# DLR-AMR/t8gpu

Hardware: AMD Instinct MI355X
Metric: M cell-updates/sec (flux+RK3 step) on Kelvin-Helmholtz AMR (higher is better)
Workload: dtype f64

## Files before the change

### include/t8gpu_hip.h

```cpp
#ifndef T8GPU_HIP_H
#define T8GPU_HIP_H

#include <stddef.h>
#include <stdint.h>

#ifdef __cplusplus
extern "C" {
#endif

#define T8GPU_FLUX_KEPES 0
#define T8GPU_FLUX_HLL 1
#define T8GPU_FLUX_HLLC 2

typedef struct T8gpuVars_f32 { float* p[5]; } T8gpuVars_f32;
typedef struct T8gpuVars_f64 { double* p[5]; } T8gpuVars_f64;

int         t8gpu_hip_abi_version(void);
int         t8gpu_hip_device_count(int* count);
int         t8gpu_hip_set_device(int device);
const char* t8gpu_hip_error_string(int code);
int         t8gpu_hip_range_push(const char* name);
int         t8gpu_hip_range_pop(void);
const char* t8gpu_hip_last_stage_kernel(void);

// ... 48 lines not shown
                                   void* stream);
int t8gpu_hip_subgrid_boundary_f64(int flux_kind, int rank, int num_faces, int num_boundary_faces,
                                   const int32_t* face_neighbors, const double* face_normals,
                                   const double* face_surfaces, T8gpuVars_f64 state, T8gpuVars_f64 fluxes,
                                   void* stream);
int t8gpu_hip_subgrid_boundary_bc_f32(int flux_kind, int rank, int num_faces, int num_boundary_faces,
                                      const int32_t* face_neighbors, const uint8_t* boundary_kinds, const float* inflow_table,
                                      const float* face_normals, const float* face_surfaces, T8gpuVars_f32 state,
                                      T8gpuVars_f32 fluxes, void* stream);
int t8gpu_hip_subgrid_boundary_bc_f64(int flux_kind, int rank, int num_faces, int num_boundary_faces,
                                      const int32_t* face_neighbors, const uint8_t* boundary_kinds, const double* inflow_table,
                                      const double* face_normals, const double* face_surfaces, T8gpuVars_f64 state,
                                      T8gpuVars_f64 fluxes, void* stream);
int t8gpu_hip_subgrid_boundary_far_f32(int flux_kind, int rank, int num_faces, int num_boundary_faces,
                                       const int32_t* face_neighbors, const uint8_t* boundary_kinds, const float* inflow_table,
                                       const float* face_normals, const float* face_surfaces, T8gpuVars_f32 state,
                                       T8gpuVars_f32 fluxes, void* stream);
int t8gpu_hip_subgrid_boundary_far_f64(int flux_kind, int rank, int num_faces, int num_boundary_faces,
                                       const int32_t* face_neighbors, const uint8_t* boundary_kinds, const double* inflow_table,
                                       const double* face_normals, const double* face_surfaces, T8gpuVars_f64 state,
                                       T8gpuVars_f64 fluxes, void* stream);

int t8gpu_hip_subgrid_rk3_stage_f32(int stage, int rank, int num_elements, T8gpuVars_f32 prev, T8gpuVars_f32 mid,
                                    T8gpuVars_f32 out, T8gpuVars_f32 fluxes, const float* volumes, float delta_t,
                                    void* stream);
int t8gpu_hip_subgrid_rk3_stage_f64(int stage, int rank, int num_elements, T8gpuVars_f64 prev, T8gpuVars_f64 mid,
                                    T8gpuVars_f64 out, T8gpuVars_f64 fluxes, const double* volumes, double delta_t,
                                    void* stream);

typedef struct T8gpuPlainPlan {
  const int32_t*  elem_off;
  const int32_t*  halo_off;
  const int32_t*  face_off;
  const int32_t*  halo_ids;
  const uint32_t* face_lr;
  const void*     face_geo;
  const int32_t*  face_orig;
  const int32_t*  csr_off;
  const uint16_t* csr_ent;
  const int32_t*  tile_order;
  int32_t ntiles, n_interior_tiles, max_elems, max_halo, max_faces, ell_width;
  const uint16_t* ell;
  const uint16_t* geo_idx;
  const void*     geo_table;
  int32_t n_geo;
  int32_t max_slots;
  int32_t n_deep_tiles;
  int32_t n_slots_addressed;
  const int32_t* tile_desc;
  int32_t n_patch_tiles[3];
  int32_t patch_dim;
  int32_t n_irregular_tiles[3];
  const void*    ghost_buf;
  const int32_t* send_map;
  const int32_t* send_list;
  void*          send_buf;
  int32_t        n_owned;
  int32_t        reserved7;
  const void*    inflow;
  int32_t        has_open_faces;
  int32_t        has_farfield_faces;
} T8gpuPlainPlan;

#define T8GPU_INFLOW_WORDS 16
int t8gpu_hip_plain_inflow_table_f32(const float* states, int num_states, float* table, void* stream);
int t8gpu_hip_plain_inflow_table_f64(const double* states, int num_states, double* table, void* stream);

int t8gpu_hip_plain_fused_stage_f32(int flux_kind, int stage, const T8gpuPlainPlan* plan, int tile_begin,
                                    int tile_count, T8gpuVars_f32 prev, T8gpuVars_f32 mid, T8gpuVars_f32 out,
                                    const float* volume, float delta_t, float* speed_estimates, void* stream);
int t8gpu_hip_plain_fused_stage_f64(int flux_kind, int stage, const T8gpuPlainPlan* plan, int tile_begin,
                                    int tile_count, T8gpuVars_f64 prev, T8gpuVars_f64 mid, T8gpuVars_f64 out,
                                    const double* volume, double delta_t, double* speed_estimates, void* stream);

int t8gpu_hip_plain_fused_stage_planar_f32(int flux_kind, int stage, const T8gpuPlainPlan* plan, int tile_begin,
                                           int tile_count, T8gpuVars_f32 prev, T8gpuVars_f32 mid, T8gpuVars_f32 out,
                                           const float* volume, float delta_t, float* speed_estimates, void* stream, int planar);
int t8gpu_hip_plain_fused_stage_planar_f64(int flux_kind, int stage, const T8gpuPlainPlan* plan, int tile_begin,
                                           int tile_count, T8gpuVars_f64 prev, T8gpuVars_f64 mid, T8gpuVars_f64 out,
                                           const double* volume, double delta_t, double* speed_estimates, void* stream, int planar);

int t8gpu_hip_plain_persistent_accepts(const T8gpuPlainPlan* plan, int flux_kind, int float_size, int tile_count);
int t8gpu_hip_plain_needs_csr(const T8gpuPlainPlan* plan);
int t8gpu_hip_plain_geo_frames_f32(void* geo_table, int n_geo, void* stream);
int t8gpu_hip_plain_geo_frames_f64(void* geo_table, int n_geo, void* stream);

int t8gpu_hip_halo_pack_f32(int n_send, int cells_per_element, const int32_t* send_idx, T8gpuVars_f32 state,
                            float* sendbuf, void* stream);
int t8gpu_hip_halo_pack_f64(int n_send, int cells_per_element, const int32_t* send_idx, T8gpuVars_f64 state,
                            double* sendbuf, void* stream);
int t8gpu_hip_halo_unpack_f32(int num_ghosts, int first_ghost_slot, int cells_per_element, const float* recvbuf,
                              T8gpuVars_f32 state, void* stream);
int t8gpu_hip_halo_unpack_f64(int num_ghosts, int first_ghost_slot, int cells_per_element, const double* recvbuf,
                              T8gpuVars_f64 state, void* stream);

int t8gpu_hip_comm_unique_id(char* id128);
int t8gpu_hip_comm_create(const char* id128, int rank, int nranks, void** comm);
int t8gpu_hip_comm_destroy(void* comm);
int t8gpu_hip_comm_abort(void* comm);
int t8gpu_hip_stream_wait(void* stream, double timeout_s);
int t8gpu_hip_runtime_versions(int out4[4]);

typedef struct T8gpuHalo {
  int32_t num_elements, num_ghosts, n_peers, n_send;
  int32_t cells_per_element, reserved;
  const int32_t* peers;
  const int32_t* send_off;
  const int32_t* recv_off;
  const int32_t* send_idx;
  void* sendbuf;
  void* recvbuf;
  void* comm;
} T8gpuHalo;

int t8gpu_hip_halo_exchange_f32(const T8gpuHalo* halo, T8gpuVars_f32 state, void* stream);
int t8gpu_hip_halo_exchange_f64(const T8gpuHalo* halo, T8gpuVars_f64 state, void* stream);

int t8gpu_hip_plain_stepper_create(const T8gpuPlainPlan* plan, const T8gpuHalo* halo_or_null, void** stepper);
int t8gpu_hip_plain_stepper_destroy(void* stepper);
int t8gpu_hip_plain_stepper_iterate_f32(void* stepper, int flux_kind, float* planes, size_t stride, int prev, int next,
                                        float delta_t, float* speed_estimates, void* stream);
int t8gpu_hip_plain_stepper_iterate_f64(void* stepper, int flux_kind, double* planes, size_t stride, int prev, int next,
                                        double delta_t, double* speed_estimates, void* stream);
int t8gpu_hip_plain_stepper_iterate_steps_f32(void* stepper, int flux_kind, float* planes, size_t stride, int prev, int next,
                                              float delta_t, float* speed_estimates, int n_steps, void* stream);
int t8gpu_hip_plain_stepper_iterate_steps_f64(void* stepper, int flux_kind, double* planes, size_t stride, int prev, int next,
                                              double delta_t, double* speed_estimates, int n_steps, void* stream);
int t8gpu_hip_plain_stepper_graph(void* stepper, int enable, int* counts);
int t8gpu_hip_plain_stepper_timing(void* stepper, int enable);
int t8gpu_hip_stepper_set_planar(void* stepper, int mode);
int t8gpu_hip_stepper_planar(void* stepper);
int t8gpu_hip_stepper_host_profile(int reset, double* ns4, long long* calls4);
int t8gpu_hip_plain_stepper_elapsed(void* stepper, double* total_ms, int* launches);
int t8gpu_hip_plain_stepper_timed_stages(void* stepper);
int t8gpu_hip_plain_stepper_host_time(void* stepper, int reset, double* total_ms, long long* steps);

typedef struct T8gpuSubgridPlan {
  const int32_t* block_rec;
  const int32_t* bf_rec;
  int32_t num_elements, rank, max_faces_per_block, n_interior_blocks;
  int32_t n_deep_blocks;
  int32_t n_blocks_addressed;
  const int32_t* fam_rec;
  const int32_t* rest_rec;
  int32_t n_families, n_rest;
  const void*    inflow;
  int32_t        has_open_faces;
  int32_t        has_farfield_faces;
} T8gpuSubgridPlan;

int t8gpu_hip_subgrid_fused_stage_f32(int flux_kind, int stage, const T8gpuSubgridPlan* plan, int block_begin,
                                      int block_count, T8gpuVars_f32 prev, T8gpuVars_f32 mid, T8gpuVars_f32 out,
                                      const float* volumes, float delta_t, void* stream);
int t8gpu_hip_subgrid_fused_stage_f64(int flux_kind, int stage, const T8gpuSubgridPlan* plan, int block_begin,
                                      int block_count, T8gpuVars_f64 prev, T8gpuVars_f64 mid, T8gpuVars_f64 out,
                                      const double* volumes, double delta_t, void* stream);

int t8gpu_hip_subgrid_stepper_create(const T8gpuSubgridPlan* plan, const T8gpuHalo* halo_or_null, void** stepper);
int t8gpu_hip_subgrid_stepper_iterate_steps_f32(void* stepper, int flux_kind, float* planes, size_t stride, const float* volumes,
                                                int prev, int next, float delta_t, int n_steps, void* stream);
int t8gpu_hip_subgrid_stepper_iterate_steps_f64(void* stepper, int flux_kind, double* planes, size_t stride, const double* volumes,
                                                int prev, int next, double delta_t, int n_steps, void* stream);

size_t t8gpu_hip_reduce_workspace_bytes(void);
int t8gpu_hip_planes_or_bits_f32(size_t n, const float* const planes[4], uint32_t* out4, void* stream);
int t8gpu_hip_planes_or_bits_f64(size_t n, const double* const planes[4], uint32_t* out4, void* stream);
// ... 81 lines not shown
```

### t8gpu_amd/csrc/hip/fused_common.hpp

```cpp
#ifndef T8GPU_HIP_FUSED_COMMON_HPP
#define T8GPU_HIP_FUSED_COMMON_HPP

#include <hip/hip_runtime.h>

#include <cstdlib>
#include <type_traits>
#include <utility>

#include "flux_math.hpp"
#include "t8gpu_hip.h"

namespace t8gpu_hip {

inline int device_cu_count() {
  static const int n = [] {
    int             dev = 0;
    hipDeviceProp_t prop;
    if (hipGetDevice(&dev) != hipSuccess || hipGetDeviceProperties(&prop, dev) != hipSuccess) return 0;
    return prop.multiProcessorCount > 0 ? prop.multiProcessorCount : 256;
  }();
  return n;
}
inline int env_per_cu(const char* name) {
  const char* env = std::getenv(name);
// ... 203 lines not shown
}
template <class T>
T8_DEV void inflow_prim(const T8gpuPlainPlan& P, int k, Prim<T>& q) {
  const T* w = inflow_entry<T>(P, k) + 5;
  q.rho = w[0]; q.vx = w[1]; q.vy = w[2]; q.vz = w[3]; q.p = w[4]; q.beta = w[5]; q.lrho = w[6]; q.lbeta = w[7]; q.v0 = w[8];
}

template <class T>
struct vec16;
template <>
struct vec16<double> {
  using type = double2;
  static constexpr int lanes = 2;
};
template <>
struct vec16<float> {
  using type = float4;
  static constexpr int lanes = 4;
};

template <class T, int NW>
constexpr int rec_words() {
  return sizeof(T) == 8 ? (NW > 5 ? 10 : 6) : 12;
}

template <class T>
size_t record_lds(int kind, size_t words, size_t records) {
  const size_t rec = kind == 0 ? rec_words<T, kPrimWords>() : rec_words<T, 5>();
  return sizeof(T) * (words + rec * records) + lds_log_table<T>(kind);
}

template <class T, int NW>
T8_DEV void rec_store(T* rec, const T* w) {
  using V         = typename vec16<T>::type;
  constexpr int L = vec16<T>::lanes;
#pragma unroll
  for (int c = 0; c + L <= NW; c += L) {
    V v;
    T* vv = reinterpret_cast<T*>(&v);
#pragma unroll
    for (int j = 0; j < L; j++) vv[j] = w[c + j];
    *reinterpret_cast<V*>(rec + c) = v;
  }
#pragma unroll
  for (int c = NW / L * L; c < NW; c++) rec[c] = w[c];
}

template <class T, int NW>
T8_DEV void rec_load(const T* rec, T* w) {
  using V         = typename vec16<T>::type;
  constexpr int L = vec16<T>::lanes;
#pragma unroll
  for (int c = 0; c + L <= NW; c += L) {
    const V  v  = *reinterpret_cast<const V*>(rec + c);
    const T* vv = reinterpret_cast<const T*>(&v);
#pragma unroll
    for (int j = 0; j < L; j++) w[c + j] = vv[j];
  }
#pragma unroll
  for (int c = NW / L * L; c < NW; c++) w[c] = rec[c];
}

template <class T>
T8_DEV void prim_words(const T s[5], T w[kPrimWords], const double* logtab) {
  const Prim<T> q = prim_from_state<T, sizeof(T) == 8>(s, logtab);
  w[0] = q.rho; w[1] = q.vx; w[2] = q.vy; w[3] = q.vz; w[4] = q.p; w[5] = q.beta; w[6] = q.lrho; w[7] = q.lbeta; w[8] = q.v0;
}
template <class T>
T8_DEV void words_prim(const T w[kPrimWords], Prim<T>& q) {
  q.rho = w[0]; q.vx = w[1]; q.vy = w[2]; q.vz = w[3]; q.p = w[4]; q.beta = w[5]; q.lrho = w[6]; q.lbeta = w[7]; q.v0 = w[8];
}

constexpr int kPrimWordsPlanar = 8;
template <class T>
T8_DEV void prim_words_planar(const T s[4], T w[kPrimWordsPlanar], const double* logtab) {
  const Prim<T> q = prim_from_state_planar<T, sizeof(T) == 8>(s, logtab);
  w[0] = q.rho; w[1] = q.vx; w[2] = q.vy; w[3] = q.p; w[4] = q.beta; w[5] = q.lrho; w[6] = q.lbeta; w[7] = q.v0;
}
template <class T>
T8_DEV void words_prim_planar(const T w[kPrimWordsPlanar], Prim<T>& q) {
  q.rho = w[0]; q.vx = w[1]; q.vy = w[2]; q.p = w[3]; q.beta = w[4]; q.lrho = w[5]; q.lbeta = w[6]; q.v0 = w[7];
}

template <class T>
int plain_persistent_stage(int kind, int stage, const T8gpuPlainPlan* plan, int tile_begin, int tile_count, FVars<T> prev,
                           FVars<T> mid, FVars<T> out, const T* volume, T dt, T* speed, hipStream_t stream);

template <class T>
int plain_patch_stage(int kind, int stage, const T8gpuPlainPlan* plan, int patch_begin, int patch_count, int tile_begin, int tile_count,
                      FVars<T> prev, FVars<T> mid, FVars<T> out, const T* volume, T dt, T* speed, bool persistent, bool planar,
                      hipStream_t stream);

template <class T>
int plain_patch3_stage(int kind, int stage, const T8gpuPlainPlan* plan, int tile_begin, int tile_count, FVars<T> prev, FVars<T> mid,
                       FVars<T> out, const T* volume, T dt, T* speed, bool persistent, bool irregular, hipStream_t stream);

template <class T>
int plain_patch3_both_stage(int kind, int stage, const T8gpuPlainPlan* plan, int reg_begin, int reg_count, int irr_begin, int irr_count,
                            FVars<T> prev, FVars<T> mid, FVars<T> out, const T* volume, T dt, T* speed, hipStream_t stream);

}

#endif
```

### t8gpu_amd/csrc/hip/kernels_compat.hip

```cpp
#include <hip/hip_runtime.h>

#pragma clang fp contract(off)

#include "flux_math.hpp"
#include "fused_common.hpp"
#include "stage_kernel_note.hpp"
#include "t8gpu_hip.h"
#include "t8gpu_host.h"

namespace t8gpu_hip {

template <class T>
struct Vars {
  T* p[5];
};

template <class T>
T8_DEV void load5(const Vars<T>& v, size_t i, T s[5]) {
#pragma unroll
  for (int k = 0; k < 5; k++) s[k] = v.p[k][i];
}

template <class T>
T8_DEV void gadd(T* addr, T v) {
// ... 405 lines not shown
  if (rank == 3) {
    if (kind == 0) T8_INNER(0, 3); else if (kind == 1) T8_INNER(1, 3); else T8_INNER(2, 3);
  } else {
    if (kind == 0) T8_INNER(0, 2); else if (kind == 1) T8_INNER(1, 2); else T8_INNER(2, 2);
  }
#undef T8_INNER
  return launch_status();
}

template <class T, bool WALL, class V>
int subgrid_faces(int kind, int rank, int F, int count, const int32_t* fn, const int32_t* idx, const int32_t* ld,
                  const int32_t* off, const T* normals, const T* areas, V st, V fl, void* stream) {
  if (count <= 0) return 0;
  if ((rank != 2 && rank != 3) || (kind < 0 || kind > 2)) return static_cast<int>(hipErrorInvalidValue);
  hipStream_t s   = static_cast<hipStream_t>(stream);
  const int   fpb = rank == 3 ? 4 : 16;
  const dim3  block(64), grid((count + fpb - 1) / fpb);
#define T8_FACES(K, R)                                                                                              \
  hipLaunchKernelGGL((k_subgrid_faces<T, K, R, WALL>), grid, block, 0, s, F, count, fn, idx, ld, off, normals, areas, \
                     mk<T>(st), mk<T>(fl))
  if (rank == 3) {
    if (kind == 0) T8_FACES(0, 3); else if (kind == 1) T8_FACES(1, 3); else T8_FACES(2, 3);
  } else {
    if (kind == 0) T8_FACES(0, 2); else if (kind == 1) T8_FACES(1, 2); else T8_FACES(2, 2);
  }
#undef T8_FACES
  return launch_status();
}

template <class T, class V>
int subgrid_boundary_bc(int kind, int rank, int F, int B, const int32_t* fn, const uint8_t* kinds, const T* inflow, const T* normals,
                        const T* areas, V st, V fl, void* stream) {
  if (!kinds) return subgrid_faces<T, true, V>(kind, rank, F, B, fn, nullptr, nullptr, nullptr, normals, areas, st, fl, stream);
  if (B <= 0) return 0;
  if ((rank != 2 && rank != 3) || (kind < 0 || kind > 2)) return static_cast<int>(hipErrorInvalidValue);
  hipStream_t s   = static_cast<hipStream_t>(stream);
  const int   fpb = rank == 3 ? 4 : 16;
  const dim3  block(64), grid((B + fpb - 1) / fpb);
#define T8_BC(K, R) \
  hipLaunchKernelGGL((k_subgrid_boundary_bc<T, K, R>), grid, block, 0, s, F, B, fn, kinds, inflow, normals, areas, mk<T>(st), mk<T>(fl))
  if (rank == 3) {
    if (kind == 0) T8_BC(0, 3); else if (kind == 1) T8_BC(1, 3); else T8_BC(2, 3);
  } else {
    if (kind == 0) T8_BC(0, 2); else if (kind == 1) T8_BC(1, 2); else T8_BC(2, 2);
  }
#undef T8_BC
  return launch_status();
}

template <class T, class V>
int subgrid_boundary_far(int kind, int rank, int F, int B, const int32_t* fn, const uint8_t* kinds, const T* inflow, const T* normals,
                         const T* areas, V st, V fl, void* stream) {
  if (!kinds) return subgrid_faces<T, true, V>(kind, rank, F, B, fn, nullptr, nullptr, nullptr, normals, areas, st, fl, stream);
  if (B <= 0) return 0;
  if ((rank != 2 && rank != 3) || (kind < 0 || kind > 2)) return static_cast<int>(hipErrorInvalidValue);
  hipStream_t s   = static_cast<hipStream_t>(stream);
  const int   fpb = rank == 3 ? 4 : 16;
  const dim3  block(64), grid((B + fpb - 1) / fpb);
#define T8_FAR(K, R) \
  hipLaunchKernelGGL((k_subgrid_boundary_far<T, K, R>), grid, block, 0, s, F, B, fn, kinds, inflow, normals, areas, mk<T>(st), mk<T>(fl))
  if (rank == 3) {
    if (kind == 0) T8_FAR(0, 3); else if (kind == 1) T8_FAR(1, 3); else T8_FAR(2, 3);
  } else {
    if (kind == 0) T8_FAR(0, 2); else if (kind == 1) T8_FAR(1, 2); else T8_FAR(2, 2);
  }
#undef T8_FAR
  return launch_status();
}

}

namespace t8gpu_hip {
StageKernelNote& stage_kernel_note() {
  static thread_local StageKernelNote note = {{0}, -1};
  return note;
}
}

using namespace t8gpu_hip;

extern "C" {

const char* t8gpu_hip_last_stage_kernel(void) { return stage_kernel_note().name; }
int t8gpu_hip_abi_version(void) { return 13; }
int t8gpu_hip_device_count(int* count) { return static_cast<int>(hipGetDeviceCount(count)); }
int t8gpu_hip_set_device(int device) { return static_cast<int>(hipSetDevice(device)); }
const char* t8gpu_hip_error_string(int code) {
  if (code >= 10000) return "RCCL error (code - 10000 is the ncclResult_t)";
  return hipGetErrorString(static_cast<hipError_t>(code));
}

#define T8_DEFINE_COMPAT(SUF, T, V)                                                                                  \
  int t8gpu_hip_flux_faces_##SUF(int kind, int F, int ndim, const int32_t* fn, const int32_t* idx, const T* normals, \
                                 const T* areas, V st, V fl, T* speed, void* stream) {                               \
    return flux_faces<T, V>(kind, F, ndim, fn, idx, normals, areas, st, fl, speed, stream);                          \
  }                                                                                                                  \
  int t8gpu_hip_flux_boundary_##SUF(int kind, int F, int B, int ndim, const int32_t* fn, const T* normals,           \
                                    const T* areas, V st, V fl, T* speed, void* stream) {                            \
    return flux_boundary<T, V>(kind, F, B, ndim, fn, normals, areas, st, fl, speed, stream);                         \
  }                                                                                                                  \
  int t8gpu_hip_flux_boundary_bc_##SUF(int kind, int F, int B, int ndim, const int32_t* fn, const uint8_t* kinds,       \
                                       const T* inflow, const T* normals, const T* areas, V st, V fl, T* speed,        \
                                       void* stream) {                                                                 \
    return flux_boundary_bc<T, V>(kind, F, B, ndim, fn, kinds, inflow, normals, areas, st, fl, speed, stream);         \
  }                                                                                                                  \
  int t8gpu_hip_rk3_stage_##SUF(int stage, int N, V prev, V mid, V out, V fl, const T* volume, T dt, void* stream) { \
    return rk_stage<T, 1, V>(stage, N < 0 ? 0 : (size_t)N, prev, mid, out, fl, volume, dt, stream);                  \
  }                                                                                                                  \
  int t8gpu_hip_subgrid_inner_##SUF(int kind, int rank, int N, V st, V fl, const T* volumes, void* stream) {         \
    return subgrid_inner<T, V>(kind, rank, N, st, fl, volumes, stream);                                              \
  }                                                                                                                  \
  int t8gpu_hip_subgrid_outer_##SUF(int kind, int rank, int F, const int32_t* fn, const int32_t* idx,                \
                                    const int32_t* ld, const int32_t* off, const T* normals, const T* areas, V st,   \
                                    V fl, void* stream) {                                                            \
    return subgrid_faces<T, false, V>(kind, rank, F, F, fn, idx, ld, off, normals, areas, st, fl, stream);           \
  }                                                                                                                  \
  int t8gpu_hip_subgrid_boundary_##SUF(int kind, int rank, int F, int B, const int32_t* fn, const T* normals,        \
                                       const T* areas, V st, V fl, void* stream) {                                   \
    return subgrid_faces<T, true, V>(kind, rank, F, B, fn, nullptr, nullptr, nullptr, normals, areas, st, fl,        \
                                     stream);                                                                        \
  }                                                                                                                  \
  int t8gpu_hip_subgrid_boundary_bc_##SUF(int kind, int rank, int F, int B, const int32_t* fn, const uint8_t* kinds,  \
                                          const T* inflow, const T* normals, const T* areas, V st, V fl,             \
                                          void* stream) {                                                            \
    return subgrid_boundary_bc<T, V>(kind, rank, F, B, fn, kinds, inflow, normals, areas, st, fl, stream);           \
  }                                                                                                                  \
  int t8gpu_hip_subgrid_boundary_far_##SUF(int kind, int rank, int F, int B, const int32_t* fn, const uint8_t* kinds, \
                                           const T* inflow, const T* normals, const T* areas, V st, V fl,            \
                                           void* stream) {                                                           \
    return subgrid_boundary_far<T, V>(kind, rank, F, B, fn, kinds, inflow, normals, areas, st, fl, stream);          \
  }                                                                                                                  \
  int t8gpu_hip_subgrid_rk3_stage_##SUF(int stage, int rank, int N, V prev, V mid, V out, V fl, const T* volumes,    \
                                        T dt, void* stream) {                                                        \
    if (rank == 3) return rk_stage<T, 64, V>(stage, (size_t)(N < 0 ? 0 : N) * 64, prev, mid, out, fl, volumes, dt, stream); \
    if (rank == 2) return rk_stage<T, 16, V>(stage, (size_t)(N < 0 ? 0 : N) * 16, prev, mid, out, fl, volumes, dt, stream); \
    return static_cast<int>(hipErrorInvalidValue);                                                                   \
  }

T8_DEFINE_COMPAT(f32, float, T8gpuVars_f32)
T8_DEFINE_COMPAT(f64, double, T8gpuVars_f64)

}
```

### t8gpu_amd/csrc/hip/kernels_fused_patch.hip

```cpp
#include "fused_common.hpp"
#include "fused_tile_body.hpp"
#include "patch_common.hpp"
#include "stage_kernel_note.hpp"

namespace t8gpu_hip {

template <class T, int KIND, int STAGE, bool NT, bool PLANAR = false>
T8_DEV void plain_patch_body(const T8gpuPlainPlan& P, int tile_begin, int tile_count, int wg, int nwg, int chunk, const FVars<T>& prev,
                             const FVars<T>& src, const FVars<T>& out, const T* __restrict__ vol, T dt, T* __restrict__ speed) {
  static_assert(!PLANAR || KIND == 0, "the planar form exists for KEPES");
  constexpr int NV  = PLANAR ? 4 : 5;
  constexpr int NW  = KIND == 0 ? (PLANAR ? kPrimWordsPlanar : kPrimWords) : 5;
  constexpr int REC = rec_words<T, NW>();
  auto pl = [](int c) { return PLANAR && c == 3 ? 4 : c; };
  extern __shared__ __attribute__((aligned(16))) double lds_raw[];
  T* const  ff = reinterpret_cast<T*>(lds_raw);
  T* const  pe = ff + NV * kPatchFF;
  constexpr bool kTab = sizeof(T) == 8 && KIND == 0;
  double* const lt = reinterpret_cast<double*>(pe + REC * 320);
  const int tid = threadIdx.x;

  const int G = nwg, xcd = wg & 7, jw = wg >> 3;
  const int nxcd = G < 8 ? G : 8, nx = (G - xcd + 7) >> 3;
  const int per = tile_count / nxcd, rem = tile_count % nxcd;
  const int x0   = tile_begin + xcd * per + (xcd < rem ? xcd : rem);
  int       tend = x0 + per + (xcd < rem ? 1 : 0);
  int       t    = x0 + (chunk > 0 ? jw * chunk : jw);
  if (chunk > 0 && t + chunk < tend) tend = t + chunk;
  if (xcd >= nxcd || t >= tend) return;
  if (kTab) {
    lt[tid] = kLogTab[tid];
    __syncthreads();
  }

  int ci = 0, cj = 0;
#pragma unroll
  for (int b = 0; b < 4; b++) {
    ci |= ((tid >> (2 * b)) & 1) << b;
    cj |= ((tid >> (2 * b + 1)) & 1) << b;
  }
  const int  rx   = ci < 15 ? patch_morton(ci + 1, cj) : 272 + cj;
  const int  ry   = cj < 15 ? patch_morton(ci, cj + 1) : 304 + ci;
  const int  a_mx = ci > 0 ? patch_morton(ci - 1, cj) : 512 + cj;
  const int  a_my = cj > 0 ? 256 + patch_morton(ci, cj - 1) : 528 + ci;
  const bool yfirst_lane = patch_ctz4(cj) >= patch_ctz4(ci);
  const int  wv = __builtin_amdgcn_readfirstlane(tid >> 6), ln = tid & 63;
  auto role = [&](int it) { return (wv + it) & 3; };
  const int  hl      = ln;
  const bool minus_y = ln >= 16;
  const int  m_l = 256 + (minus_y ? 32 : 0) + (ln & 15);
  const int  m_r = minus_y ? patch_morton(ln & 15, 0) : patch_morton(0, ln & 15);

  typedef int int8v __attribute__((ext_vector_type(8)));
  struct Desc {
    int    e0, h0, fbase, flags;
    double area, vol;
  };
  auto load_desc = [&](int tt) {
    const size_t k = static_cast<size_t>(tt < tend ? tt : tend - 1);
    const int8v  r = *reinterpret_cast<const __attribute__((address_space(4))) int8v*>(
        reinterpret_cast<const __attribute__((address_space(4))) char*>(reinterpret_cast<uintptr_t>(P.tile_desc)) + 32 * k);
    Desc d;
    d.e0 = r[0]; d.h0 = r[2]; d.fbase = r[4]; d.flags = r[5];
    d.area = __hiloint2double(r[7], r[6]);
    d.vol  = __hiloint2double(r[3], r[1]);
    return d;
  };
  struct Pre {
    T s0[NV], sh[NV];
  };
  auto prefetch = [&](const Desc& d, int hslot, bool first, bool halo_wave) {
    Pre p;
#pragma unroll
    for (int k = 0; k < NV; k++) p.s0[k] = at32<T>(src.p[pl(k)], static_cast<unsigned>(d.e0 + tid));
    if (!PLANAR && halo_wave && first && P.ghost_buf) {
#pragma unroll
      for (int k = 0; k < NV; k++) p.sh[k] = ghost_window_load<T>(P, src, hslot, pl(k));
    } else if (halo_wave) {
#pragma unroll
      for (int k = 0; k < NV; k++) p.sh[k] = at32<T>(src.p[pl(k)], static_cast<unsigned>(hslot));
    } else {
#pragma unroll
      for (int k = 0; k < NV; k++) p.sh[k] = T(0);
    }
    return p;
  };

  const int stride = chunk > 0 ? 1 : nx;
  Desc      d0 = load_desc(t), d1 = load_desc(t + stride);
  int       hs_a = role(0) == 3 ? P.halo_ids[d0.h0 + hl] : 0, hs_b = role(1) == 3 ? P.halo_ids[d1.h0 + hl] : 0;
  Pre       cur = prefetch(d0, hs_a, true, role(0) == 3);
  int       it  = 0;
  T         res[NV];
#pragma unroll
  for (int k = 0; k < NV; k++) res[k] = T(0);
  int       res_e  = -1;
  __builtin_amdgcn_s_waitcnt(0);

  for (; t < tend; t += stride, it++) {
    const bool halo_wave = role(it) == 3, minus_lane = role(it) == 0 && ln < 32;
    const Desc d2   = load_desc(t + 2 * stride);
    const int  hs_c = role(it + 2) == 3 ? P.halo_ids[d2.h0 + hl] : 0;
    Pre        nxt;
    if (t + stride < tend) nxt = prefetch(d1, hs_b, false, role(it + 1) == 3);
    const int e = d0.e0 + tid;
    T         pv[NV];
#pragma unroll
    for (int k = 0; k < NV; k++) pv[k] = T(0);
    if (STAGE > 1) {
#pragma unroll
      for (int k = 0; k < NV; k++) pv[k] = stream_load<NT>(&at32<T>(prev.p[pl(k)], static_cast<unsigned>(e)));
    }
    const T volume = (d0.flags & 0x400) ? static_cast<T>(d0.vol) : at32<T>(vol, static_cast<unsigned>(e));
    const T area   = static_cast<T>(d0.area);

    T mine[NW];
    if constexpr (PLANAR) {
      prim_words_planar<T>(cur.s0, mine, lt);
    } else if constexpr (KIND == 0) {
      prim_words<T>(cur.s0, mine, lt);
    } else {
#pragma unroll
      for (int k = 0; k < 5; k++) mine[k] = cur.s0[k];
    }
    rec_store<T, NW>(pe + tid * REC, mine);
    if (halo_wave) {
      T w[NW];
      if constexpr (PLANAR) {
        prim_words_planar<T>(cur.sh, w, lt);
      } else if constexpr (KIND == 0) {
        prim_words<T>(cur.sh, w, lt);
      } else {
#pragma unroll
        for (int k = 0; k < 5; k++) w[k] = cur.sh[k];
      }
      rec_store<T, NW>(pe + (256 + hl) * REC, w);
    }
    if (res_e >= 0) {
#pragma unroll
      for (int k = 0; k < NV; k++) stream_store<NT>(&at32<T>(out.p[pl(k)], static_cast<unsigned>(res_e)), res[k]);
    }
    __syncthreads();

    auto face = [&](bool y, const T* wl, const T* wr, T* g, T& spd) {
      if constexpr (PLANAR)
        patch_face_planar<T>(y, wl, wr, area, g, spd);
      else
        patch_face<T, KIND, NW>(y, wl, wr, area, g, spd);
    };
    T gy[NV];
    {
      T wr[NW], g[NV], sx, sy;
      rec_load<T, NW>(pe + rx * REC, wr);
      face(false, mine, wr, g, sx);
#pragma unroll
      for (int k = 0; k < NV; k++) ff[k * kPatchFF + tid] = g[k];
      rec_load<T, NW>(pe + ry * REC, wr);
      face(true, mine, wr, gy, sy);
#pragma unroll
      for (int k = 0; k < NV; k++) ff[k * kPatchFF + 256 + tid] = gy[k];
      if (speed) {
        T* const sp = speed + d0.fbase + 2 * tid;
        if ((d0.fbase & 1) == 0 || sizeof(T) == 4) {
          using V2 = typename vec2<T>::type;
          V2 v;
          v.x = sx;
          v.y = sy;
          *reinterpret_cast<V2*>(sp) = v;
        } else {
          sp[0] = sx;
          sp[1] = sy;
        }
      }
    }
    if (minus_lane) {
      T wl[NW], wr[NW], g[NV], sm;
      rec_load<T, NW>(pe + m_l * REC, wl);
      rec_load<T, NW>(pe + m_r * REC, wr);
      face(minus_y, wl, wr, g, sm);
#pragma unroll
      for (int k = 0; k < NV; k++) ff[k * kPatchFF + 512 + ln] = g[k];
    }
    __syncthreads();

    const bool yfirst = tid == 0 ? (d0.flags & 1) != 0 : yfirst_lane;
    const int  a1 = yfirst ? a_my : a_mx, a2 = yfirst ? a_mx : a_my;
    T          acc[NV];
#pragma unroll
    for (int k = 0; k < NV; k++) {
      acc[k] = __builtin_fma(T(1), ff[k * kPatchFF + a1], T(0));
      acc[k] = __builtin_fma(T(1), ff[k * kPatchFF + a2], acc[k]);
      acc[k] = __builtin_fma(T(-1), ff[k * kPatchFF + tid], acc[k]);
      acc[k] = __builtin_fma(T(-1), gy[k], acc[k]);
    }
    const T scale = (d0.flags & 0x400) ? rk_scale(dt, static_cast<T>(d0.vol)) : dt / volume;
#pragma unroll
    for (int k = 0; k < NV; k++) res[k] = rk_stage_update<T, STAGE>(pv[k], cur.s0[k], scale, acc[k]);
    res_e = e;

    cur  = nxt;
    d0   = d1;
    d1   = d2;
    hs_b = hs_c;
  }
  if (res_e >= 0) {
#pragma unroll
    for (int k = 0; k < NV; k++) stream_store<NT>(&at32<T>(out.p[pl(k)], static_cast<unsigned>(res_e)), res[k]);
    if constexpr (!PLANAR)
      if (P.send_map) ghost_window_send<T>(P, res_e, res);
  }
}

template <class T, int KIND, int STAGE, bool NT, bool PLANAR = false>
__global__ __launch_bounds__(256, sizeof(T) == 8 ? 3 : 5) void k_plain_patch(T8gpuPlainPlan P, int tile_begin, int tile_count, int chunk, FVars<T> prev,
                                                                                FVars<T> src, FVars<T> out, const T* __restrict__ vol, T dt,
                                                                                T* __restrict__ speed) {
  plain_patch_body<T, KIND, STAGE, NT, PLANAR>(P, tile_begin, tile_count, blockIdx.x, gridDim.x, chunk, prev, src, out, vol, dt, speed);
}

template <class T, int KIND, int STAGE, bool NT, bool OPEN = false, bool PLANAR = false>
__global__ __launch_bounds__(256, sizeof(T) == 8 ? 3 : 5) void k_plain_stage(T8gpuPlainPlan P, int patch_begin, int patch_count, int patch_wgs, int chunk,
                                                                                int tile_begin, int tile_count, FVars<T> prev, FVars<T> src,
                                                                                FVars<T> out, const T* __restrict__ vol, T dt,
                                                                                T* __restrict__ speed) {
  const int b = blockIdx.x;
  if (b < patch_wgs) {
    plain_patch_body<T, KIND, STAGE, NT, PLANAR>(P, patch_begin, patch_count, b, patch_wgs, chunk, prev, src, out, vol, dt, speed);
  } else {
    const int pos = tile_begin + xcd_position(b - patch_wgs, tile_count);
    plain_tile_body<T, KIND, STAGE, true, 2, false, OPEN>(P, pos, prev, src, out, vol, dt, speed);
  }
}

template <class T>
int plain_patch_stage(int kind, int stage, const T8gpuPlainPlan* plan, int patch_begin, int patch_count, int tile_begin, int tile_count,
                      FVars<T> prev, FVars<T> mid, FVars<T> out, const T* volume, T dt, T* speed, bool persistent, bool planar,
                      hipStream_t stream) {
  if (patch_count <= 0) return tile_count > 0 ? -1 : 0;
  const bool shared_gpu = plan->n_interior_tiles < plan->ntiles && patch_count + (tile_count > 0 ? tile_count : 0) < plan->ntiles;
  if (!plan->tile_desc) return static_cast<int>(hipErrorInvalidValue);
  if (!plan_planes_fit_32bit<T>(plan)) return static_cast<int>(hipErrorInvalidValue);
  if (plan->ghost_buf || plan->send_map || !persistent || kind != 0) planar = false;
  size_t lds = record_lds<T>(kind, static_cast<size_t>(planar ? 4 : 5) * kPatchFF, 320);
  if (tile_count > 0 && plan->has_farfield_faces) return -1;
  if (tile_count > 0) {
    if (!plain_tiles_pipelined(plan) || plan->max_faces > 512 || !plan->geo_idx || !plan->geo_table || plan->n_geo <= 0) return -1;
    const int    nw       = kind == 0 ? kPrimWords : 5;
    const size_t tab      = lds_log_table<T>(kind);
    const size_t lds_tile = sizeof(T) * (static_cast<size_t>(nw) * plan_slots(*plan) + static_cast<size_t>(5) * 256) + (tab ? tab + 16 : 0);
    if (lds_tile > lds) lds = lds_tile;
    if (sizeof(T) == 8 && 3 * lds > static_cast<size_t>(156) * 1024) return -1;
  }
  const int cus = device_cu_count();
  if (cus == 0) return static_cast<int>(hipErrorInvalidDevice);
  if (plan->ghost_buf || plan->send_map) persistent = false;
  const int  per_cu    = sizeof(T) == 8 ? 3 : 5;
  const int  resident  = cus * per_cu;
  int chunk = 0;
  if (persistent && shared_gpu && patch_count >= resident) chunk = 3;
  int patch_wgs = (!persistent || patch_count < resident) ? patch_count : resident;
  if (chunk > 0) {
    const int share = (patch_count + 7) / 8;
    patch_wgs       = 8 * ((share + chunk - 1) / chunk);
  }
  const dim3 grid(patch_wgs + (tile_count > 0 ? tile_count : 0)), block(256);
  const bool nt = stream_hint(plan->n_slots_addressed, sizeof(T));
  return dispatch(
      [&](auto K, auto S, auto NT, auto MIXED, auto OPEN, auto PLANAR) {
        constexpr bool PL = PLANAR && K == 0;
        if constexpr (MIXED) {
          note_stage_kernel<T>(patch_count + tile_count, "k_plain_stage", K, S, NT, OPEN, PL);
          return launch(&k_plain_stage<T, K, S, NT, OPEN, PL>, grid, block, lds, stream, *plan, patch_begin, patch_count, patch_wgs, chunk,
                        tile_begin, tile_count, prev, mid, out, volume, dt, speed);
        } else {
          note_stage_kernel<T>(patch_count, "k_plain_patch", K, S, NT, PL);
          return launch(&k_plain_patch<T, K, S, NT, PL>, grid, block, lds, stream, *plan, patch_begin, patch_count, chunk, prev, mid, out, volume,
                        dt, speed);
        }
      },
      kind, stage, nt, tile_count > 0, tile_count > 0 && plan->has_open_faces, planar);
}

template int plain_patch_stage<float>(int, int, const T8gpuPlainPlan*, int, int, int, int, FVars<float>, FVars<float>, FVars<float>,
                                      const float*, float, float*, bool, bool, hipStream_t);
template int plain_patch_stage<double>(int, int, const T8gpuPlainPlan*, int, int, int, int, FVars<double>, FVars<double>, FVars<double>,
                                       const double*, double, double*, bool, bool, hipStream_t);

}
```

### t8gpu_amd/csrc/hip/patch_common.hpp

```cpp
#ifndef T8GPU_HIP_PATCH_COMMON_HPP
#define T8GPU_HIP_PATCH_COMMON_HPP

#include "fused_common.hpp"

namespace t8gpu_hip {

template <class T>
T8_DEV const T& at32(const T* base, unsigned i) {
  return *reinterpret_cast<const T*>(reinterpret_cast<const char*>(base) + i * static_cast<unsigned>(sizeof(T)));
}
template <class T>
T8_DEV T& at32(T* base, unsigned i) {
  return *reinterpret_cast<T*>(reinterpret_cast<char*>(base) + i * static_cast<unsigned>(sizeof(T)));
}

template <class T>
bool plan_planes_fit_32bit(const T8gpuPlainPlan* plan) {
  return plan->n_slots_addressed > 0 && static_cast<unsigned long long>(plan->n_slots_addressed) * sizeof(T) < (1ull << 32);
}

constexpr int kPatchFF = 544;

T8_DEV int patch_morton(int i, int j) {
  int t = 0;
#pragma unroll
  for (int b = 0; b < 4; b++) t |= (((i >> b) & 1) << (2 * b)) | (((j >> b) & 1) << (2 * b + 1));
  return t;
}
T8_DEV int patch_ctz4(int v) { return v == 0 ? 4 : __builtin_ctz(static_cast<unsigned>(v)); }

template <class T>
T8_DEV void frame_in(bool y, T vx, T vy, T vz, T& u, T& v, T& w) {
  u = y ? vy : vx;
  v = y ? vx : -vz;
  w = y ? -vz : vy;
}
template <class T>
T8_DEV void frame_out(bool y, const T f[5], T g[5]) {
  g[0] = f[0];
  g[1] = y ? f[2] : f[1];
  g[2] = y ? f[1] : f[3];
  g[3] = y ? -f[3] : -f[2];
  g[4] = f[4];
}

template <class T, int KIND, int NW>
T8_DEV void patch_face(bool y, const T* wl, const T* wr, T area, T g[5], T& spd) {
  T f[5];
  if (KIND == 0) {
    Prim<T> L, R;
    words_prim<T>(wl, L);
    words_prim<T>(wr, R);
    T uL, vL, wL, uR, vR, wR;
    frame_in<T>(y, L.vx, L.vy, L.vz, uL, vL, wL);
    frame_in<T>(y, R.vx, R.vy, R.vz, uR, vR, wR);
    kepes_core<T>(L, R, uL, vL, wL, uR, vR, wR, area, f, spd);
  } else {
    T a[5], b[5];
    a[0] = wl[0]; a[4] = wl[4];
    b[0] = wr[0]; b[4] = wr[4];
    frame_in<T>(y, wl[1], wl[2], wl[3], a[1], a[2], a[3]);
    frame_in<T>(y, wr[1], wr[2], wr[3], b[1], b[2], b[3]);
    if (KIND == 2)
      hllc_fast<T>(a, b, f, spd);
    else
      hll_fast<T>(a, b, f, spd);
#pragma unroll
    for (int k = 0; k < 5; k++) f[k] = area * f[k];
  }
  frame_out<T>(y, f, g);
}

template <class T>
T8_DEV void patch_face_planar(bool y, const T* wl, const T* wr, T area, T g[4], T& spd) {
  Prim<T> L, R;
  words_prim_planar<T>(wl, L);
  words_prim_planar<T>(wr, R);
  T f[4];
  kepes_core_planar<T>(L, R, y ? L.vy : L.vx, y ? L.vx : L.vy, y ? R.vy : R.vx, y ? R.vx : R.vy, area, f, spd);
  g[0] = f[0];
  g[1] = y ? f[2] : f[1];
  g[2] = y ? f[1] : f[2];
  g[3] = f[3];
}

template <class T>
T8_DEV void frame_in3(int axis, T vx, T vy, T vz, T& u, T& v, T& w) {
  u = axis == 0 ? vx : (axis == 1 ? vy : vz);
  v = axis == 0 ? -vz : (axis == 1 ? vx : vy);
  w = axis == 0 ? vy : (axis == 1 ? -vz : -vx);
}
template <class T>
T8_DEV void frame_out3(int axis, const T f[5], T g[5]) {
  g[0] = f[0];
  g[1] = axis == 0 ? f[1] : (axis == 1 ? f[2] : -f[3]);
  g[2] = axis == 0 ? f[3] : (axis == 1 ? f[1] : f[2]);
  g[3] = axis == 0 ? -f[2] : (axis == 1 ? -f[3] : f[1]);
  g[4] = f[4];
}
template <class T, int KIND, int NW>
T8_DEV void patch_face3(int axis, const T* wl, const T* wr, T area, T g[5], T& spd) {
  T f[5];
  if (KIND == 0) {
    Prim<T> L, R;
// ... 85 lines not shown
```

### t8gpu_amd/hip.py

```python
import ctypes as C
import os

import numpy as np

from . import build as _build

ABI_VERSION = 13
KEPES, HLL, HLLC = 0, 1, 2


class Vars32(C.Structure):
    _fields_ = [("p", C.c_void_p * 5)]


class Vars64(C.Structure):
    _fields_ = [("p", C.c_void_p * 5)]


class T8gpuHipError(RuntimeError):
    pass


_lib = None


def lib():
    global _lib
    if _lib is None:
        import torch
        path = _build.HIP_LIB
        if not os.path.exists(path):
            raise T8gpuHipError(f"{path} is missing: run `python -m t8gpu_amd.build` (hipcc --offload-arch=gfx950). "
                                "There is no CPU fallback for the hot path.")
        _lib = C.CDLL(path)
        _lib.t8gpu_hip_abi_version.restype = C.c_int
        if _lib.t8gpu_hip_abi_version() != ABI_VERSION:
            got, _lib = _lib.t8gpu_hip_abi_version(), None
            raise T8gpuHipError(f"{path} has ABI version {got}, this package needs {ABI_VERSION}: rebuild it "
                                "(`python -m t8gpu_amd.build`)")
        _lib.t8gpu_hip_error_string.restype = C.c_char_p
        _lib.t8gpu_hip_error_string.argtypes = [C.c_int]
    return _lib


def check(code):
    if code != 0:
        raise T8gpuHipError(f"t8gpu_hip call failed: {code} ({lib().t8gpu_hip_error_string(code).decode()})")


def suffix(dtype):
    import torch
    if dtype in (torch.float32, np.float32):
        return "f32"
    if dtype in (torch.float64, np.float64):
        return "f64"
    raise TypeError(f"float_type must be float32 or float64, got {dtype}")


def vars_of(planes, step=0):
    import torch
    cls = Vars32 if planes.dtype == torch.float32 else Vars64
    v = cls()
    for k in range(5):
        v.p[k] = planes[5 * step + k].data_ptr()
    return v


def ptr(t):
    return None if t is None else C.c_void_p(t.data_ptr())


def stream_ptr(stream=None):
    import torch
    s = stream if stream is not None else torch.cuda.current_stream()
    return C.c_void_p(s.cuda_stream)


def fscalar(dtype, x):
    import torch
    return C.c_float(x) if dtype == torch.float32 else C.c_double(x)


def call(name, dtype, *args):
    fn = getattr(lib(), f"{name}_{suffix(dtype)}")
    fn.restype = C.c_int
    check(fn(*args))
```

Measured before the change: 14500.

## Split planar f64 LDS records into 16-byte chunks and allow four patch WGs per CU

For the planar f64 KEPES patch kernel, primitive records in LDS move to a chunked structure-of-arrays layout of 16-byte double2 pieces, which packs them without padding and gives conflict-friendlier wide accesses. All state planes are now addressed from one base pointer plus a uniform stride, with a runtime check that the planes are equally spaced, which may free scalar registers. When the LDS footprint fits a quarter of the CU budget, launch bounds and residency go from three to four workgroups per CU. Register pressure from the tighter launch bound may cause spills, and there is an env override to keep three.

```diff
diff --git a/include/t8gpu_hip.h b/include/t8gpu_hip.h
--- a/include/t8gpu_hip.h
+++ b/include/t8gpu_hip.h
@@ -154,6 +154,7 @@
 
 int t8gpu_hip_plain_persistent_accepts(const T8gpuPlainPlan* plan, int flux_kind, int float_size, int tile_count);
 int t8gpu_hip_plain_needs_csr(const T8gpuPlainPlan* plan);
+int t8gpu_hip_plain_patch_lds_bytes(const T8gpuPlainPlan* plan, int flux_kind, int float_size, int planar);
 int t8gpu_hip_plain_geo_frames_f32(void* geo_table, int n_geo, void* stream);
 int t8gpu_hip_plain_geo_frames_f64(void* geo_table, int n_geo, void* stream);
 
diff --git a/t8gpu_amd/csrc/hip/fused_common.hpp b/t8gpu_amd/csrc/hip/fused_common.hpp
--- a/t8gpu_amd/csrc/hip/fused_common.hpp
+++ b/t8gpu_amd/csrc/hip/fused_common.hpp
@@ -309,6 +309,27 @@
   q.rho = w[0]; q.vx = w[1]; q.vy = w[2]; q.p = w[3]; q.beta = w[4]; q.lrho = w[5]; q.lbeta = w[6]; q.v0 = w[7];
 }
 
+constexpr int kSplitChunkBytes = 16;
+template <int RECORDS>
+T8_DEV void rec_split_store(double* recs, int off0, const double w[kPrimWordsPlanar]) {
+#pragma unroll
+  for (int c = 0; c < 4; c++) {
+    double2 v;
+    v.x = w[2 * c];
+    v.y = w[2 * c + 1];
+    *reinterpret_cast<double2*>(reinterpret_cast<char*>(recs) + off0 + c * (kSplitChunkBytes * RECORDS)) = v;
+  }
+}
+template <int RECORDS>
+T8_DEV void rec_split_load(const double* recs, int off0, double w[kPrimWordsPlanar]) {
+#pragma unroll
+  for (int c = 0; c < 4; c++) {
+    const double2 v = *reinterpret_cast<const double2*>(reinterpret_cast<const char*>(recs) + off0 + c * (kSplitChunkBytes * RECORDS));
+    w[2 * c]     = v.x;
+    w[2 * c + 1] = v.y;
+  }
+}
+
 template <class T>
 int plain_persistent_stage(int kind, int stage, const T8gpuPlainPlan* plan, int tile_begin, int tile_count, FVars<T> prev,
                            FVars<T> mid, FVars<T> out, const T* volume, T dt, T* speed, hipStream_t stream);
diff --git a/t8gpu_amd/csrc/hip/kernels_compat.hip b/t8gpu_amd/csrc/hip/kernels_compat.hip
--- a/t8gpu_amd/csrc/hip/kernels_compat.hip
+++ b/t8gpu_amd/csrc/hip/kernels_compat.hip
@@ -511,7 +511,7 @@
 extern "C" {
 
 const char* t8gpu_hip_last_stage_kernel(void) { return stage_kernel_note().name; }
-int t8gpu_hip_abi_version(void) { return 13; }
+int t8gpu_hip_abi_version(void) { return 14; }
 int t8gpu_hip_device_count(int* count) { return static_cast<int>(hipGetDeviceCount(count)); }
 int t8gpu_hip_set_device(int device) { return static_cast<int>(hipSetDevice(device)); }
 const char* t8gpu_hip_error_string(int code) {
diff --git a/t8gpu_amd/csrc/hip/kernels_fused_patch.hip b/t8gpu_amd/csrc/hip/kernels_fused_patch.hip
--- a/t8gpu_amd/csrc/hip/kernels_fused_patch.hip
+++ b/t8gpu_amd/csrc/hip/kernels_fused_patch.hip
@@ -11,7 +11,8 @@
   static_assert(!PLANAR || KIND == 0, "the planar form exists for KEPES");
   constexpr int NV  = PLANAR ? 4 : 5;
   constexpr int NW  = KIND == 0 ? (PLANAR ? kPrimWordsPlanar : kPrimWords) : 5;
-  constexpr int REC = rec_words<T, NW>();
+  constexpr bool SPLIT = PLANAR && sizeof(T) == 8;
+  constexpr int  REC = SPLIT ? kPrimWordsPlanar : rec_words<T, NW>();
   auto pl = [](int c) { return PLANAR && c == 3 ? 4 : c; };
   extern __shared__ __attribute__((aligned(16))) double lds_raw[];
   T* const  ff = reinterpret_cast<T*>(lds_raw);
@@ -19,6 +20,31 @@
   constexpr bool kTab = sizeof(T) == 8 && KIND == 0;
   double* const lt = reinterpret_cast<double*>(pe + REC * 320);
   const int tid = threadIdx.x;
+  auto rec_at = [](int r) { return SPLIT ? kSplitChunkBytes * r : r * REC; };
+  auto store_rec = [&](int h, const T* w) {
+    if constexpr (SPLIT)
+      rec_split_store<320>(reinterpret_cast<double*>(pe), h, reinterpret_cast<const double*>(w));
+    else
+      rec_store<T, NW>(pe + h, w);
+  };
+  auto load_rec = [&](int h, T* w) {
+    if constexpr (SPLIT)
+      rec_split_load<320>(reinterpret_cast<const double*>(pe), h, reinterpret_cast<double*>(w));
+    else
+      rec_load<T, NW>(pe + h, w);
+  };
+
+  using GT = __attribute__((address_space(1))) T;
+  long pstride = 0;
+  if constexpr (SPLIT) pstride = reinterpret_cast<const char*>(src.p[1]) - reinterpret_cast<const char*>(src.p[0]);
+  auto plane = [&](const FVars<T>& v, int k) -> T* {
+    if constexpr (SPLIT) {
+      uintptr_t a = reinterpret_cast<uintptr_t>(v.p[0]) + static_cast<uintptr_t>(pl(k) * pstride);
+      return (T*)reinterpret_cast<GT*>(a);
+    } else {
+      return v.p[pl(k)];
+    }
+  };
 
   const int G = nwg, xcd = wg & 7, jw = wg >> 3;
   const int nxcd = G < 8 ? G : 8, nx = (G - xcd + 7) >> 3;
@@ -39,8 +65,9 @@
     ci |= ((tid >> (2 * b)) & 1) << b;
     cj |= ((tid >> (2 * b + 1)) & 1) << b;
   }
-  const int  rx   = ci < 15 ? patch_morton(ci + 1, cj) : 272 + cj;
-  const int  ry   = cj < 15 ? patch_morton(ci, cj + 1) : 304 + ci;
+  const int  rx   = rec_at(ci < 15 ? patch_morton(ci + 1, cj) : 272 + cj);
+  const int  ry   = rec_at(cj < 15 ? patch_morton(ci, cj + 1) : 304 + ci);
+  const int  rme  = rec_at(tid);
   const int  a_mx = ci > 0 ? patch_morton(ci - 1, cj) : 512 + cj;
   const int  a_my = cj > 0 ? 256 + patch_morton(ci, cj - 1) : 528 + ci;
   const bool yfirst_lane = patch_ctz4(cj) >= patch_ctz4(ci);
@@ -48,8 +75,8 @@
   auto role = [&](int it) { return (wv + it) & 3; };
   const int  hl      = ln;
   const bool minus_y = ln >= 16;
-  const int  m_l = 256 + (minus_y ? 32 : 0) + (ln & 15);
-  const int  m_r = minus_y ? patch_morton(ln & 15, 0) : patch_morton(0, ln & 15);
+  const int  m_l = rec_at(256 + (minus_y ? 32 : 0) + (ln & 15));
+  const int  m_r = rec_at(minus_y ? patch_morton(ln & 15, 0) : patch_morton(0, ln & 15));
 
   typedef int int8v __attribute__((ext_vector_type(8)));
   struct Desc {
@@ -72,13 +99,13 @@
   auto prefetch = [&](const Desc& d, int hslot, bool first, bool halo_wave) {
     Pre p;
 #pragma unroll
-    for (int k = 0; k < NV; k++) p.s0[k] = at32<T>(src.p[pl(k)], static_cast<unsigned>(d.e0 + tid));
+    for (int k = 0; k < NV; k++) p.s0[k] = at32<T>(plane(src, k), static_cast<unsigned>(d.e0 + tid));
     if (!PLANAR && halo_wave && first && P.ghost_buf) {
 #pragma unroll
       for (int k = 0; k < NV; k++) p.sh[k] = ghost_window_load<T>(P, src, hslot, pl(k));
     } else if (halo_wave) {
 #pragma unroll
-      for (int k = 0; k < NV; k++) p.sh[k] = at32<T>(src.p[pl(k)], static_cast<unsigned>(hslot));
+      for (int k = 0; k < NV; k++) p.sh[k] = at32<T>(plane(src, k), static_cast<unsigned>(hslot));
     } else {
 #pragma unroll
       for (int k = 0; k < NV; k++) p.sh[k] = T(0);
@@ -98,6 +125,7 @@
   __builtin_amdgcn_s_waitcnt(0);
 
   for (; t < tend; t += stride, it++) {
+    if constexpr (SPLIT) asm volatile("" : "+s"(pstride));
     const bool halo_wave = role(it) == 3, minus_lane = role(it) == 0 && ln < 32;
     const Desc d2   = load_desc(t + 2 * stride);
     const int  hs_c = role(it + 2) == 3 ? P.halo_ids[d2.h0 + hl] : 0;
@@ -109,7 +137,7 @@
     for (int k = 0; k < NV; k++) pv[k] = T(0);
     if (STAGE > 1) {
 #pragma unroll
-      for (int k = 0; k < NV; k++) pv[k] = stream_load<NT>(&at32<T>(prev.p[pl(k)], static_cast<unsigned>(e)));
+      for (int k = 0; k < NV; k++) pv[k] = stream_load<NT>(&at32<T>(plane(prev, k), static_cast<unsigned>(e)));
     }
     const T volume = (d0.flags & 0x400) ? static_cast<T>(d0.vol) : at32<T>(vol, static_cast<unsigned>(e));
     const T area   = static_cast<T>(d0.area);
@@ -123,7 +151,7 @@
 #pragma unroll
       for (int k = 0; k < 5; k++) mine[k] = cur.s0[k];
     }
-    rec_store<T, NW>(pe + tid * REC, mine);
+    store_rec(rme, mine);
     if (halo_wave) {
       T w[NW];
       if constexpr (PLANAR) {
@@ -134,11 +162,11 @@
 #pragma unroll
         for (int k = 0; k < 5; k++) w[k] = cur.sh[k];
       }
-      rec_store<T, NW>(pe + (256 + hl) * REC, w);
+      store_rec(rec_at(256 + hl), w);
     }
     if (res_e >= 0) {
 #pragma unroll
-      for (int k = 0; k < NV; k++) stream_store<NT>(&at32<T>(out.p[pl(k)], static_cast<unsigned>(res_e)), res[k]);
+      for (int k = 0; k < NV; k++) stream_store<NT>(&at32<T>(plane(out, k), static_cast<unsigned>(res_e)), res[k]);
     }
     __syncthreads();
 
@@ -151,11 +179,11 @@
     T gy[NV];
     {
       T wr[NW], g[NV], sx, sy;
-      rec_load<T, NW>(pe + rx * REC, wr);
+      load_rec(rx, wr);
       face(false, mine, wr, g, sx);
 #pragma unroll
       for (int k = 0; k < NV; k++) ff[k * kPatchFF + tid] = g[k];
-      rec_load<T, NW>(pe + ry * REC, wr);
+      load_rec(ry, wr);
       face(true, mine, wr, gy, sy);
 #pragma unroll
       for (int k = 0; k < NV; k++) ff[k * kPatchFF + 256 + tid] = gy[k];
@@ -175,8 +203,8 @@
     }
     if (minus_lane) {
       T wl[NW], wr[NW], g[NV], sm;
-      rec_load<T, NW>(pe + m_l * REC, wl);
-      rec_load<T, NW>(pe + m_r * REC, wr);
+      load_rec(m_l, wl);
+      load_rec(m_r, wr);
       face(minus_y, wl, wr, g, sm);
 #pragma unroll
       for (int k = 0; k < NV; k++) ff[k * kPatchFF + 512 + ln] = g[k];
@@ -205,21 +233,26 @@
   }
   if (res_e >= 0) {
 #pragma unroll
-    for (int k = 0; k < NV; k++) stream_store<NT>(&at32<T>(out.p[pl(k)], static_cast<unsigned>(res_e)), res[k]);
+    for (int k = 0; k < NV; k++) stream_store<NT>(&at32<T>(plane(out, k), static_cast<unsigned>(res_e)), res[k]);
     if constexpr (!PLANAR)
       if (P.send_map) ghost_window_send<T>(P, res_e, res);
   }
 }
 
+template <class T, bool PLANAR>
+constexpr int patch_wgs_per_cu() {
+  return sizeof(T) == 8 ? (PLANAR ? 4 : 3) : 5;
+}
+
 template <class T, int KIND, int STAGE, bool NT, bool PLANAR = false>
-__global__ __launch_bounds__(256, sizeof(T) == 8 ? 3 : 5) void k_plain_patch(T8gpuPlainPlan P, int tile_begin, int tile_count, int chunk, FVars<T> prev,
+__global__ __launch_bounds__(256, (patch_wgs_per_cu<T, PLANAR>())) void k_plain_patch(T8gpuPlainPlan P, int tile_begin, int tile_count, int chunk, FVars<T> prev,
                                                                                 FVars<T> src, FVars<T> out, const T* __restrict__ vol, T dt,
                                                                                 T* __restrict__ speed) {
   plain_patch_body<T, KIND, STAGE, NT, PLANAR>(P, tile_begin, tile_count, blockIdx.x, gridDim.x, chunk, prev, src, out, vol, dt, speed);
 }
 
 template <class T, int KIND, int STAGE, bool NT, bool OPEN = false, bool PLANAR = false>
-__global__ __launch_bounds__(256, sizeof(T) == 8 ? 3 : 5) void k_plain_stage(T8gpuPlainPlan P, int patch_begin, int patch_count, int patch_wgs, int chunk,
+__global__ __launch_bounds__(256, (patch_wgs_per_cu<T, PLANAR>())) void k_plain_stage(T8gpuPlainPlan P, int patch_begin, int patch_count, int patch_wgs, int chunk,
                                                                                 int tile_begin, int tile_count, FVars<T> prev, FVars<T> src,
                                                                                 FVars<T> out, const T* __restrict__ vol, T dt,
                                                                                 T* __restrict__ speed) {
@@ -233,6 +266,21 @@
 }
 
 template <class T>
+bool planes_equally_spaced(const FVars<T>& v, const FVars<T>& ref) {
+  const ptrdiff_t d = reinterpret_cast<const char*>(ref.p[1]) - reinterpret_cast<const char*>(ref.p[0]);
+  for (int k = 0; k < 4; k++)
+    if (reinterpret_cast<const char*>(v.p[k + 1]) - reinterpret_cast<const char*>(v.p[k]) != d) return false;
+  return true;
+}
+
+template <class T>
+size_t mixed_tile_lds(int kind, const T8gpuPlainPlan* plan) {
+  const int    nw  = kind == 0 ? kPrimWords : 5;
+  const size_t tab = lds_log_table<T>(kind);
+  return sizeof(T) * (static_cast<size_t>(nw) * plan_slots(*plan) + static_cast<size_t>(5) * 256) + (tab ? tab + 16 : 0);
+}
+
+template <class T>
 int plain_patch_stage(int kind, int stage, const T8gpuPlainPlan* plan, int patch_begin, int patch_count, int tile_begin, int tile_count,
                       FVars<T> prev, FVars<T> mid, FVars<T> out, const T* volume, T dt, T* speed, bool persistent, bool planar,
                       hipStream_t stream) {
@@ -241,20 +289,23 @@
   if (!plan->tile_desc) return static_cast<int>(hipErrorInvalidValue);
   if (!plan_planes_fit_32bit<T>(plan)) return static_cast<int>(hipErrorInvalidValue);
   if (plan->ghost_buf || plan->send_map || !persistent || kind != 0) planar = false;
-  size_t lds = record_lds<T>(kind, static_cast<size_t>(planar ? 4 : 5) * kPatchFF, 320);
+  if (planar && sizeof(T) == 8 && !(planes_equally_spaced(mid, mid) && planes_equally_spaced(out, mid) && (stage == 1 || planes_equally_spaced(prev, mid))))
+    planar = false;
+  size_t lds = patch_lds<T>(kind, planar);
+  const bool planar64 = planar && sizeof(T) == 8;
   if (tile_count > 0 && plan->has_farfield_faces) return -1;
   if (tile_count > 0) {
     if (!plain_tiles_pipelined(plan) || plan->max_faces > 512 || !plan->geo_idx || !plan->geo_table || plan->n_geo <= 0) return -1;
-    const int    nw       = kind == 0 ? kPrimWords : 5;
-    const size_t tab      = lds_log_table<T>(kind);
-    const size_t lds_tile = sizeof(T) * (static_cast<size_t>(nw) * plan_slots(*plan) + static_cast<size_t>(5) * 256) + (tab ? tab + 16 : 0);
+    const size_t lds_tile = mixed_tile_lds<T>(kind, plan);
     if (lds_tile > lds) lds = lds_tile;
     if (sizeof(T) == 8 && 3 * lds > static_cast<size_t>(156) * 1024) return -1;
   }
+  static const int per_cu_env = env_per_cu("T8GPU_PATCH_WGS");
+  const bool       four       = planar64 && lds <= kLdsQuarterCU && per_cu_env != 3;
   const int cus = device_cu_count();
   if (cus == 0) return static_cast<int>(hipErrorInvalidDevice);
   if (plan->ghost_buf || plan->send_map) persistent = false;
-  const int  per_cu    = sizeof(T) == 8 ? 3 : 5;
+  const int  per_cu    = sizeof(T) == 8 ? (four ? 4 : 3) : 5;
   const int  resident  = cus * per_cu;
   int chunk = 0;
   if (persistent && shared_gpu && patch_count >= resident) chunk = 3;
@@ -281,9 +332,21 @@
       kind, stage, nt, tile_count > 0, tile_count > 0 && plan->has_open_faces, planar);
 }
 
+size_t plain_patch_window(int kind, int float_size, bool planar, const T8gpuPlainPlan* tiles) {
+  if (kind != 0) planar = false;
+  const size_t lds  = float_size == 8 ? patch_lds<double>(kind, planar) : patch_lds<float>(kind, planar);
+  const size_t tile = !tiles ? 0 : float_size == 8 ? mixed_tile_lds<double>(kind, tiles) : mixed_tile_lds<float>(kind, tiles);
+  return tile > lds ? tile : lds;
+}
+
 template int plain_patch_stage<float>(int, int, const T8gpuPlainPlan*, int, int, int, int, FVars<float>, FVars<float>, FVars<float>,
                                       const float*, float, float*, bool, bool, hipStream_t);
 template int plain_patch_stage<double>(int, int, const T8gpuPlainPlan*, int, int, int, int, FVars<double>, FVars<double>, FVars<double>,
                                        const double*, double, double*, bool, bool, hipStream_t);
 
 }
+
+extern "C" int t8gpu_hip_plain_patch_lds_bytes(const T8gpuPlainPlan* plan, int flux_kind, int float_size, int planar) {
+  if (flux_kind < 0 || flux_kind > 2 || (float_size != 4 && float_size != 8)) return -1;
+  return static_cast<int>(t8gpu_hip::plain_patch_window(flux_kind, float_size, planar != 0, plan));
+}
diff --git a/t8gpu_amd/csrc/hip/patch_common.hpp b/t8gpu_amd/csrc/hip/patch_common.hpp
--- a/t8gpu_amd/csrc/hip/patch_common.hpp
+++ b/t8gpu_amd/csrc/hip/patch_common.hpp
@@ -20,6 +20,14 @@
 }
 
 constexpr int kPatchFF = 544;
+
+template <class T>
+size_t patch_lds(int kind, bool planar) {
+  if (planar && kind == 0 && sizeof(T) == 8)
+    return sizeof(T) * 4 * kPatchFF + sizeof(T) * kPrimWordsPlanar * 320 + lds_log_table<T>(kind);
+  return record_lds<T>(kind, static_cast<size_t>(planar ? 4 : 5) * kPatchFF, 320);
+}
+constexpr size_t kLdsQuarterCU = 160 * 1024 / 4;
 
 T8_DEV int patch_morton(int i, int j) {
   int t = 0;
diff --git a/t8gpu_amd/hip.py b/t8gpu_amd/hip.py
--- a/t8gpu_amd/hip.py
+++ b/t8gpu_amd/hip.py
@@ -5,7 +5,7 @@
 
 from . import build as _build
 
-ABI_VERSION = 13
+ABI_VERSION = 14
 KEPES, HLL, HLLC = 0, 1, 2
 
 
```

Measured after the change: 15080 (median of 6 runs). 4.0% higher.
